# tum-pbs/Solver-in-the-Loop

Measured on AMD Instinct MI355X. Metric: sim-steps/s, SOL-32 training (karman-2d 128x64, fwd+bwd+Adam), higher is better.
Workload: dtype f32 (fp16x3 split MFMA in 32-ch convs); 1 GPU; karman-2d 128x64 SOL-32, batch 6 Re values per GPU (BASELINE configs[2]); global_batch=6, msteps=32, parallelism=dp1

## Files before the change

solver-in-the-loop_amd/csrc/conv5x5.hip:

```cpp
#include "common.hpp"
#include <stdlib.h>

namespace {

typedef float f32x4 __attribute__((ext_vector_type(4)));

__host__ __device__ inline int pad_in(int c) { return c <= 4 ? 4 : 32; }
__host__ __device__ inline int pad_out(int c) { return c <= 16 ? 16 : 32; }

__global__ void k_pack(const float* __restrict__ w, float* __restrict__ packed, int cin, int cout, int mode) {
    const int IP = pad_in(cin), OP = pad_out(cout);
    const int total = 25 * OP * IP;
    for (int e = blockIdx.x * blockDim.x + threadIdx.x; e < total; e += gridDim.x * blockDim.x) {
        const int i = e % IP, o = (e / IP) % OP, tap = e / (IP * OP);
        float v = 0.f;
        if (i < cin && o < cout) {
            if (mode == SOL_CONV_FWD) v = w[(tap * cin + i) * cout + o];
            else v = w[((24 - tap) * cout + o) * cin + i];
        }
        packed[e] = v;
    }
}

template <int CIN, int NT, bool MASK = false>
// ... 707 lines not shown
    __syncthreads();
    while (gr < gr_end) {
        const int gnext = next_row(gr + 1);
        if (gnext < gr_end) load_row(gnext);
        const bool valid = row_valid(gr);
        const float* xs = smem + cur * bufsz;
        const float* zs = xs + (W + 4) * CPX;
        if (active_wave) {
            for (int p0 = 0; p0 < W; p0 += 4) {
                const int px = p0 + g;
                float bv;
                if constexpr (COUT > 4) bv = zs[px * CPZ + tc * 16 + li];
                else bv = li < 4 ? zs[px * CPZ + li] : 0.f;
                if (dy == 2 && ta == 0) bsum += bv;
                if (valid) {
#pragma unroll
                    for (int d = 0; d < 5; ++d) {
                        float av;
                        if constexpr (CI == 32) av = xs[(px + d) * CPX + ta * 16 + li];
                        else av = li < 4 ? xs[(px + d) * CPX + li] : 0.f;
                        acc[d] = __builtin_amdgcn_mfma_f32_16x16x4f32(av, bv, acc[d], 0, 0, 0);
                    }
                }
            }
        }
        if (gnext < gr_end) store_row(smem + (cur ^ 1) * bufsz);
        __syncthreads();
        cur ^= 1;
        gr = gnext;
    }
    if (!active_wave) return;
    float* pw = a.partial + (size_t)blk * (25 * IP * OP);
#pragma unroll
    for (int d = 0; d < 5; ++d) {
        const int tap = dy * 5 + d;
#pragma unroll
        for (int r = 0; r < 4; ++r) {
            const int ci = ta * 16 + 4 * g + r, co = tc * 16 + li;
            float* dst = &pw[(tap * IP + ci) * OP + co];
            *dst = a.overwrite ? acc[d][r] : *dst + acc[d][r];
        }
    }
    if (dy == 2 && ta == 0) {
        bsum += __shfl_xor(bsum, 16, 64);
        bsum += __shfl_xor(bsum, 32, 64);
        if (g == 0) {
            float* pb = a.partial + (size_t)a.nblk * (25 * IP * OP) + (size_t)blk * OP;
            pb[tc * 16 + li] = a.overwrite ? bsum : pb[tc * 16 + li] + bsum;
        }
    }
}

typedef float f32x16 __attribute__((ext_vector_type(16)));

__global__ void __launch_bounds__(256) k_conv5x5_bww32(BwArgs a) {
    constexpr int W = 64, STG = (W + 4) * 32 + W * 32;
    extern __shared__ __align__(16) float smem[];
    const int tid = threadIdx.x, lane = tid & 63, wave = tid >> 6;
    const int c = lane & 31, kpx = lane >> 5;
    const int H = a.H;
    const int dy = blockIdx.x % 5, blk = blockIdx.x / 5;
    f32x16 acc[5];
#pragma unroll
    for (int d = 0; d < 5; ++d)
#pragma unroll
        for (int r = 0; r < 16; ++r) acc[d][r] = 0.f;
    float bsum = 0.f;
    const int R = a.nseg * a.B * H, RPS = a.B * H;
    const int gr_end = min((blk + 1) * a.rb, R);
    auto row_valid = [&](int gr) { const int y = gr % H, yy = y + dy - 2; return yy >= 0 && yy < H; };
    auto next_row = [&](int gr) { while (gr < gr_end && !(dy == 2 || row_valid(gr))) ++gr; return gr; };
    float4 xr[3], zr[2];
    auto load_row = [&](int gr) {
        const int seg = gr / RPS, grs = gr - seg * RPS;
        const int b = grs / H, y = grs - b * H, yy = y + dy - 2;
        const bool valid = yy >= 0 && yy < H;
        const float4* gx = reinterpret_cast<const float4*>(a.x + (size_t)seg * a.x_seg) + (size_t)(b * H + (valid ? yy : 0)) * W * 8;
#pragma unroll
        for (int n = 0; n < 3; ++n) {
            const int e = tid + n * 256, px = e >> 3, c4 = e & 7, xx = px - 2;
            xr[n] = make_float4(0.f, 0.f, 0.f, 0.f);
            if (valid && px < W + 4 && xx >= 0 && xx < W) xr[n] = gx[xx * 8 + c4];
        }
        const float4* gz = reinterpret_cast<const float4*>(a.dz + (size_t)seg * a.dz_seg) + (size_t)(b * H + y) * W * 8;
#pragma unroll
        for (int n = 0; n < 2; ++n) zr[n] = gz[tid + n * 256];
    };
    auto store_row = [&](float* buf) {
#pragma unroll
        for (int n = 0; n < 3; ++n) {
            const int e = tid + n * 256;
            if (e < (W + 4) * 8) reinterpret_cast<float4*>(buf)[e] = xr[n];
        }
        float4* zs4 = reinterpret_cast<float4*>(buf + (W + 4) * 32);
#pragma unroll
        for (int n = 0; n < 2; ++n) zs4[tid + n * 256] = zr[n];
    };
    int gr = next_row(blk * a.rb);
    int cur = 0;
    if (gr < gr_end) { load_row(gr); store_row(smem); }
    __syncthreads();
    while (gr < gr_end) {
        const int gnext = next_row(gr + 1);
        if (gnext < gr_end) load_row(gnext);
        const bool valid = row_valid(gr);
        const float* xs = smem + cur * STG + (16 * wave + kpx) * 32 + c;
        const float* zs = smem + cur * STG + (W + 4) * 32 + (16 * wave + kpx) * 32 + c;
#pragma unroll
        for (int ks = 0; ks < 8; ++ks) {
            const float bv = zs[ks * 64];
            if (dy == 2) bsum += bv;
            if (valid) {
#pragma unroll
                for (int d = 0; d < 5; ++d)
                    acc[d] = __builtin_amdgcn_mfma_f32_32x32x2f32(xs[(2 * ks + d) * 32], bv, acc[d], 0, 0, 0);
            }
        }
        if (gnext < gr_end) store_row(smem + (cur ^ 1) * STG);
        __syncthreads();
        cur ^= 1;
        gr = gnext;
    }
    float* red = smem;
    float* pw = a.partial + (size_t)blk * (25 * 1024);
    for (int d = 0; d < 5; ++d) {
#pragma unroll
        for (int r = 0; r < 16; ++r) {
            const int row = (r & 3) + 8 * (r >> 2) + 4 * kpx;
            red[wave * 1024 + row * 32 + c] = acc[d][r];
        }
        __syncthreads();
#pragma unroll
        for (int n = 0; n < 4; ++n) {
            const int idx = tid + n * 256;
            const float v = (red[idx] + red[1024 + idx]) + (red[2048 + idx] + red[3072 + idx]);
            float* dst = &pw[(dy * 5 + d) * 1024 + idx];
            *dst = a.overwrite ? v : *dst + v;
        }
        __syncthreads();
    }
    if (dy == 2) {
        bsum += __shfl_xor(bsum, 32, 64);
        if (kpx == 0) red[wave * 32 + c] = bsum;
        __syncthreads();
        if (tid < 32) {
            float* pb = a.partial + (size_t)a.nblk * (25 * 1024) + (size_t)blk * 32;
            const float v = (red[tid] + red[32 + tid]) + (red[64 + tid] + red[96 + tid]);
            pb[tid] = a.overwrite ? v : pb[tid] + v;
        }
    }
}

template <int MODE, int MT, bool WIDE = false>
__global__ void __launch_bounds__(256) k_conv5x5_bww_thin(BwArgs a) {
    constexpr int W = 64;
    constexpr int XC = MODE == 0 ? 4 : 32, ZC = MODE == 0 ? 32 : 2;
    constexpr int XROWS = MODE == 0 ? 5 : 1, ZROWS = MODE == 0 ? 1 : 5;
    constexpr int XSZ = (W + 4) * XC;
    constexpr int ZSZ = (MODE == 0 ? W + 4 : W + 8) * ZC;
    constexpr int STG = XROWS * XSZ + ZROWS * ZSZ;
    constexpr int IP = MODE == 0 ? 16 : 32, OP = MODE == 0 ? 32 : 16;
    constexpr int XF4 = XROWS * XSZ / 4, ZF4 = ZROWS * ZSZ / 4;
    constexpr int NXR = (XF4 + 255) / 256, NZR = (ZF4 + 255) / 256;
    constexpr int NTM = MODE == 0 ? MT : 2, NTN = MODE == 0 ? 2 : 1;
    constexpr int CI0 = MT == 1 ? 3 : 4;
    typedef float bt_f4 __attribute__((ext_vector_type(4)));
    extern __shared__ __align__(16) float smem[];
    const int tid = threadIdx.x, lane = tid & 63, wave = tid >> 6;
    const int n16 = lane & 15, kq = lane >> 4;
    const int H = a.H, blk = blockIdx.x;
    const int WI = WIDE ? a.W : W, tiles = WIDE ? a.W / W : 1;
    const int rblk = WIDE ? blk / tiles : blk, x0 = WIDE ? (blk - rblk * tiles) * W : 0;
    bt_f4 acc[5][NTM][NTN];
#pragma unroll
    for (int d = 0; d < 5; ++d)
#pragma unroll
        for (int tm = 0; tm < NTM; ++tm)
#pragma unroll
            for (int tn = 0; tn < NTN; ++tn) acc[d][tm][tn] = (bt_f4){0.f, 0.f, 0.f, 0.f};
    float bsum[2] = {0.f, 0.f};
    const int R = a.nseg * a.B * H, RPS = a.B * H;
    const int gr_end = min((rblk + 1) * a.rb, R);
    float4 xr[NXR], zr[NZR];
    auto load_row = [&](int gr) {
        const int seg = gr / RPS, grs = gr - seg * RPS;
        const int b = grs / H, y = grs - b * H;
        const float* xb = a.x + (size_t)seg * a.x_seg + (size_t)b * H * WI * XC;
        const float* zb = a.dz + (size_t)seg * a.dz_seg + ((size_t)b * H * WI + x0) * ZC;
#pragma unroll
        for (int n = 0; n < NXR; ++n) {
            const int e = tid + n * 256;
            xr[n] = make_float4(0.f, 0.f, 0.f, 0.f);
            if (e < XF4) {
                const int row = e / (XSZ / 4), f = e - row * (XSZ / 4);
                const int px = f / (XC / 4), c4 = f - px * (XC / 4), xx = x0 + px - 2;
                const int yy = MODE == 0 ? y + row - 2 : y;
                if (yy >= 0 && yy < H && xx >= 0 && xx < WI) xr[n] = reinterpret_cast<const float4*>(xb + ((size_t)yy * WI + xx) * XC)[c4];
            }
        }
#pragma unroll
        for (int n = 0; n < NZR; ++n) {
            const int e = tid + n * 256;
            zr[n] = make_float4(0.f, 0.f, 0.f, 0.f);
            if (e < ZF4) {
                if (MODE == 0) {
                    if (e < W * ZC / 4) zr[n] = reinterpret_cast<const float4*>(zb + (size_t)y * WI * ZC)[e];
                } else {
                    const int row = e / (ZSZ / 4), f = e - row * (ZSZ / 4);
                    const int yy = y + 2 - row, p = 2 * f - 4;
                    if (yy >= 0 && yy < H && p >= 0 && p < W) zr[n] = reinterpret_cast<const float4*>(zb + ((size_t)yy * WI + p) * ZC)[0];
                }
            }
        }
    };
    auto store_row = [&](float* buf) {
#pragma unroll
        for (int n = 0; n < NXR; ++n) { const int e = tid + n * 256; if (e < XF4) reinterpret_cast<float4*>(buf)[e] = xr[n]; }
#pragma unroll
        for (int n = 0; n < NZR; ++n) { const int e = tid + n * 256; if (e < ZF4) reinterpret_cast<float4*>(buf + XROWS * XSZ)[e] = zr[n]; }
    };
    int gr = rblk * a.rb, cur = 0;
    if (gr < gr_end) { load_row(gr); store_row(smem); }
    __syncthreads();
    for (; gr < gr_end; ++gr) {
        if (gr + 1 < gr_end) load_row(gr + 1);
        const float* xs = smem + cur * STG;
        const float* zs = xs + XROWS * XSZ;
        if (MODE == 0) {
            int aoff[NTM];
            bool aok[NTM];
#pragma unroll
            for (int tm = 0; tm < NTM; ++tm) {
                const int i = 16 * tm + n16;
                aok[tm] = i < 5 * CI0;
                aoff[tm] = aok[tm] ? (i / CI0) * 4 + i % CI0 : 0;
            }
#pragma unroll
            for (int ks = 0; ks < 4; ++ks) {
                const int px = 16 * wave + 4 * ks + kq;
                float bv[2];
#pragma unroll
                for (int tn = 0; tn < 2; ++tn) { bv[tn] = zs[px * 32 + 16 * tn + n16]; bsum[tn] += bv[tn]; }
#pragma unroll
                for (int d = 0; d < 5; ++d) {
#pragma unroll
                    for (int tm = 0; tm < NTM; ++tm) {
                        const float av = aok[tm] ? xs[d * XSZ + px * 4 + aoff[tm]] : 0.f;
#pragma unroll
                        for (int tn = 0; tn < NTN; ++tn) acc[d][tm][tn] = __builtin_amdgcn_mfma_f32_16x16x4f32(av, bv[tn], acc[d][tm][tn], 0, 0, 0);
                    }
                }
            }
        } else {
            const int dxi = n16 >> 1, co = n16 & 1;
#pragma unroll
            for (int ks = 0; ks < 5; ++ks) {
                const int g = wave + 4 * ks;
                const bool ok = g < 17;
                const int qq = ok ? 4 * g + kq : 0;
                float av[2];
#pragma unroll
                for (int tm = 0; tm < 2; ++tm) av[tm] = ok ? xs[qq * 32 + 16 * tm + n16] : 0.f;
#pragma unroll
                for (int d = 0; d < 5; ++d) {
                    const float bv = (ok && n16 < 10) ? zs[d * ZSZ + (qq - dxi + 4) * 2 + co] : 0.f;
                    if (d == 2 && n16 < 2) bsum[0] += bv;
#pragma unroll
                    for (int tm = 0; tm < 2; ++tm) acc[d][tm][0] = __builtin_amdgcn_mfma_f32_16x16x4f32(av[tm], bv, acc[d][tm][0], 0, 0, 0);
                }
            }
        }
        if (gr + 1 < gr_end) store_row(smem + (cur ^ 1) * STG);
        __syncthreads();
        cur ^= 1;
    }
    float* red = smem;
    float* pw = a.partial + (size_t)blk * (25 * IP * OP);
    for (int d = 0; d < 5; ++d) {
#pragma unroll
        for (int tm = 0; tm < NTM; ++tm)
#pragma unroll
            for (int tn = 0; tn < NTN; ++tn)
#pragma unroll
                for (int r = 0; r < 4; ++r) red[wave * 1024 + (16 * tm + 4 * kq + r) * 32 + 16 * tn + n16] = acc[d][tm][tn][r];
        __syncthreads();
#pragma unroll
        for (int n = 0; n < 4; ++n) {
            const int idx = tid + n * 256, row = idx >> 5, col = idx & 31;
            const float v = (red[idx] + red[1024 + idx]) + (red[2048 + idx] + red[3072 + idx]);
            int tap, ci, co;
            bool keep;
            if (MODE == 0) { tap = d * 5 + row / CI0; ci = row % CI0; co = col; keep = row < 5 * CI0; }
            else { tap = d * 5 + (col >> 1); ci = row; co = col & 1; keep = col < 10; }
            if (keep) {
                float* dst = &pw[(tap * IP + ci) * OP + co];
                *dst = a.overwrite ? v : *dst + v;
            }
        }
        __syncthreads();
    }
    {
#pragma unroll
        for (int t = 0; t < 2; ++t) {
            bsum[t] += __shfl_xor(bsum[t], 16, 64);
            bsum[t] += __shfl_xor(bsum[t], 32, 64);
            if (kq == 0) red[wave * 32 + 16 * t + n16] = bsum[t];
        }
        __syncthreads();
        const int nb = MODE == 0 ? 32 : 2;
        if (tid < nb) {
            float* pb = a.partial + (size_t)a.nblk * (25 * IP * OP) + (size_t)blk * OP;
            const float v = (red[tid] + red[32 + tid]) + (red[64 + tid] + red[96 + tid]);
            pb[tid] = a.overwrite ? v : pb[tid] + v;
        }
    }
}

__global__ void k_bww_reduce(float* __restrict__ partial, float* __restrict__ dw, float* __restrict__ db,
                             int nblk, int cin, int cout, int IP, int OP, int chunk, int stride, int to_dw, int accumulate, int tt) {
    const int nw = 25 * cin * cout;
    const int e = blockIdx.x * blockDim.x + threadIdx.x;
    const int k0 = blockIdx.y * chunk * stride, k1 = min(k0 + chunk * stride, nblk);
    if (e < nw) {
        const int co = e % cout, ci = (e / cout) % cin, tap = e / (cout * cin);
        const size_t off = (size_t)(tap * IP + ci) * OP + co;
        float s = 0.f;
        for (int k = k0; k < k1; k += stride) s += partial[(size_t)k * (25 * IP * OP) + off];
        const int eo = tt ? (((tap % 5) * 5 + tap / 5) * cin + ci) * cout + co : e;
        if (to_dw) dw[eo] = accumulate ? dw[eo] + s : s;
        else partial[(size_t)k0 * (25 * IP * OP) + off] = s;
    } else if (e < nw + cout) {
        const int co = e - nw;
        float* pb = partial + (size_t)nblk * (25 * IP * OP);
        float s = 0.f;
        for (int k = k0; k < k1; k += stride) s += pb[(size_t)k * OP + co];
        if (to_dw) db[co] = accumulate ? db[co] + s : s;
        else pb[(size_t)k0 * OP + co] = s;
    }
}

struct ReduceJob { float *partial, *dw, *db; int nblk, cin, cout, IP, OP, ny, accumulate, tt; };
struct ReduceJobs { ReduceJob j[12]; };
__global__ void k_bww_reduce_jobs(ReduceJobs J, int stage2) {
    const ReduceJob& r = J.j[blockIdx.z];
    constexpr int CHUNK = 16;
    const int nw = 25 * r.cin * r.cout;
    const int e = blockIdx.x * blockDim.x + threadIdx.x;
    int k0, k1, stride, to_dw;
    if (!stage2) {
        if (r.ny <= 1 || (int)blockIdx.y >= r.ny) return;
        k0 = blockIdx.y * CHUNK; k1 = min(k0 + CHUNK, r.nblk); stride = 1; to_dw = 0;
    } else {
        if (blockIdx.y > 0) return;
        k0 = 0; k1 = r.nblk; stride = r.ny > 1 ? CHUNK : 1; to_dw = 1;
    }
    if (e < nw) {
        const int co = e % r.cout, ci = (e / r.cout) % r.cin, tap = e / (r.cout * r.cin);
        const size_t off = (size_t)(tap * r.IP + ci) * r.OP + co;
        float s = 0.f;
        for (int k = k0; k < k1; k += stride) s += r.partial[(size_t)k * (25 * r.IP * r.OP) + off];
        const int eo = r.tt ? (((tap % 5) * 5 + tap / 5) * r.cin + ci) * r.cout + co : e;
        if (to_dw) r.dw[eo] = r.accumulate ? r.dw[eo] + s : s;
        else r.partial[(size_t)k0 * (25 * r.IP * r.OP) + off] = s;
    } else if (e < nw + r.cout) {
        const int co = e - nw;
        float* pb = r.partial + (size_t)r.nblk * (25 * r.IP * r.OP);
        float s = 0.f;
        for (int k = k0; k < k1; k += stride) s += pb[(size_t)k * r.OP + co];
        if (to_dw) r.db[co] = r.accumulate ? r.db[co] + s : s;
        else pb[(size_t)k0 * r.OP + co] = s;
    }
}

int check_shape(int B, int H, int W, int cin, int cout) {
    SOL_REQUIRE(B >= 1 && H >= 1 && W >= 4, "conv5x5: bad image shape B=%d H=%d W=%d", B, H, W);
    SOL_REQUIRE((W <= 64 && 64 % W == 0 && H % (64 / W) == 0) || W % 64 == 0,
                "conv5x5: W must divide 64 (with H %% (64/W) == 0) or be a multiple of 64 (H=%d W=%d)", H, W);
    SOL_REQUIRE(cin == 4 || cin == 32, "conv5x5: input channels must be 4 (zero padded) or 32 (got %d)", cin);
    SOL_REQUIRE(cout >= 1 && cout <= 32, "conv5x5: output channels must be in [1,32] (got %d)", cout);
    return SOL_OK;
}

}

extern "C" int32_t sol_absmax_slots(void) {
    static_assert(SOL_AMAX_SLOTS == SOL_ABSMAX_SLOTS, "include/sol_hip.h and common.hpp disagree");
    return SOL_AMAX_SLOTS;
}

extern "C" size_t sol_conv5x5_packed_floats(int32_t cin, int32_t cout, int32_t ) {
    return (size_t)25 * pad_in(cin) * pad_out(cout) +
           (pad_in(cin) == 32 ? sol_conv_sb_packed_floats(pad_out(cout)) + sol_conv_sh_packed_floats(pad_out(cout)) : 0);
}

extern "C" int sol_conv5x5_pack(void* stream, const float* w_hwio, int32_t cin, int32_t cout, int32_t mode, float* packed) {
    SOL_REQUIRE(w_hwio && packed, "sol_conv5x5_pack: NULL pointer");
    SOL_REQUIRE(cin >= 1 && cin <= 32 && cout >= 1 && cout <= 32, "sol_conv5x5_pack: channels out of range");
    SOL_REQUIRE(mode == SOL_CONV_FWD || mode == SOL_CONV_BWD_DATA, "sol_conv5x5_pack: bad mode %d", mode);
    const int total = 25 * pad_in(cin) * pad_out(cout);
    SOL_LAUNCH(k_pack, dim3((total + 255) / 256), dim3(256), 0, (hipStream_t)stream, w_hwio, packed, cin, cout, mode);
    SOL_LAUNCH_CHECK();
    if (pad_in(cin) == 32) {
        if (int e = sol_conv_sb_pack((hipStream_t)stream, w_hwio, cin, cout, mode, packed + total)) return e;
        return sol_conv_sh_pack((hipStream_t)stream, w_hwio, cin, cout, mode, packed + total + sol_conv_sb_packed_floats(pad_out(cout)));
    }
    return SOL_OK;
}

extern "C" int sol_conv5x5_pack_jobs(void* stream, int32_t n, const float* const* w_hwio, const int32_t* cin, const int32_t* cout,
                                     const int32_t* mode, float* const* packed) {
    SOL_REQUIRE(n >= 1 && n <= 24 && w_hwio && cin && cout && mode && packed, "sol_conv5x5_pack_jobs: 1 <= n <= 24 jobs, no NULL array");
    const float* bi[24];
    float* bo[24];
    int ci[24], co[24], md[24];
    for (int k = 0; k < n; ++k) {
        SOL_REQUIRE(w_hwio[k] && packed[k], "sol_conv5x5_pack_jobs: NULL pointer in job %d", k);
        SOL_REQUIRE(cin[k] >= 1 && cin[k] <= 32 && cout[k] >= 1 && cout[k] <= 32, "sol_conv5x5_pack_jobs: channels out of range in job %d", k);
        SOL_REQUIRE(mode[k] == SOL_CONV_FWD || mode[k] == SOL_CONV_BWD_DATA, "sol_conv5x5_pack_jobs: bad mode %d in job %d", mode[k], k);
        bi[k] = nullptr; bo[k] = nullptr; ci[k] = cin[k]; co[k] = cout[k]; md[k] = mode[k];
    }
    return sol_pack_jobs((hipStream_t)stream, n, w_hwio, packed, bo, bi, ci, co, md, 0);
}

int sol_init_conv_kernels() {
    static std::atomic<unsigned long long> optin{0};
    return sol_lds_optin(optin, {SOL_K(k_conv5x5_r3<1>), SOL_K(k_conv5x5_r3<2>), SOL_K(k_conv5x5_c32<1>), SOL_K(k_conv5x5_c32<2>),
                                 SOL_K((k_conv5x5_r3<1, true>)), SOL_K((k_conv5x5_r3<2, true>)), SOL_K((k_conv5x5_c32<1, true>)), SOL_K((k_conv5x5_c32<2, true>))}, "conv kernels");
}

static int conv_impl(void* stream, const float* x, const float* packed, const float* bias,
                     const float* residual, const float* act_ref, float* y,
                     int32_t B, int32_t H, int32_t W, int32_t cin, int32_t cout,
                     int32_t epilogue, float slope, const uint32_t* x_absmax, uint32_t* y_absmax, int32_t WV = 0) {
    if (int e = check_shape(B, H, W, cin, cout)) return e;
    SOL_REQUIRE(x && packed && y, "sol_conv5x5: NULL pointer");
    SOL_REQUIRE(epilogue != SOL_EPI_DLRELU || act_ref, "sol_conv5x5: SOL_EPI_DLRELU needs act_ref");
    if (int e = sol_init_conv_kernels()) return e;
    ConvArgs a{};
    a.x = x; a.wp = packed; a.bias = bias; a.res = residual; a.act = act_ref; a.y = y;
    a.B = B; a.H = H; a.W = W; a.CO = cout; a.CI = cin; a.epi = epilogue; a.slope = slope; a.WV = WV;
    const bool mask = sol_conv_masked(a);
    a.TW = W < 64 ? W : 64;
    a.RPW = 64 / a.TW;
    a.tiles_x = W / a.TW;
    const int grid = B * (H / a.RPW) * a.tiles_x;
    const int CP = cin == 4 ? 4 : 36;
    size_t lds = (size_t)(a.RPW + 4) * (a.TW + 4) * CP * sizeof(float);
    if (cin == 4) {
        lds += (size_t)25 * pad_out(cout) * 4 * sizeof(float);
        if (lds < 4 * 16 * 32 * sizeof(float)) lds = 4 * 16 * 32 * sizeof(float);
    }
    const int NT = pad_out(cout) / 16;
    hipStream_t s = (hipStream_t)stream;
    const bool use_sb = sol_opt().conv_precision != 2;
    const bool use_sh = sol_opt().conv_precision == 0;
    if (use_sb) a.ymax = y_absmax;
    if (cin == 32 && W % 64 == 0 && use_sb) {
        a.wsb = packed + (size_t)25 * 32 * pad_out(cout);
        a.wsh = packed + (size_t)25 * 32 * pad_out(cout) + sol_conv_sb_packed_floats(pad_out(cout));
        a.xmax = use_sh ? x_absmax : nullptr;
        return sol_conv_sb_launch(s, a, NT, B * H * (W / 64));
    }
    if (cin == 32 && W % 64 == 0 && sol_opt().conv_r3) {
        const int ntiles = B * H * (W / 64);
        const size_t ldsr = ((size_t)3 * 2 * 68 * 32 + 2 * (size_t)5 * NT * 16 * 32) * sizeof(float);
        const int grid3 = (ntiles + 2) / 3;
        if (mask) {
            if (NT == 2) SOL_LAUNCH((k_conv5x5_r3<2, true>), dim3(grid3), dim3(768), ldsr, s, a, ntiles);
            else SOL_LAUNCH((k_conv5x5_r3<1, true>), dim3(grid3), dim3(768), ldsr, s, a, ntiles);
        } else if (NT == 2) {
            SOL_LAUNCH((k_conv5x5_r3<2>), dim3(grid3), dim3(768), ldsr, s, a, ntiles);
        } else {
            SOL_LAUNCH((k_conv5x5_r3<1>), dim3(grid3), dim3(768), ldsr, s, a, ntiles);
        }
    }
    else if (cin == 32) {
        const size_t lds32 = ((size_t)(a.RPW + 4) * (a.TW + 4) * 32 + 2 * (size_t)NT * 16 * 32) * sizeof(float);
        if (mask) {
            if (NT == 2) SOL_LAUNCH((k_conv5x5_c32<2, true>), dim3(grid), dim3(256), lds32, s, a);
            else SOL_LAUNCH((k_conv5x5_c32<1, true>), dim3(grid), dim3(256), lds32, s, a);
        } else if (NT == 2) {
            SOL_LAUNCH((k_conv5x5_c32<2>), dim3(grid), dim3(256), lds32, s, a);
        } else {
            SOL_LAUNCH((k_conv5x5_c32<1>), dim3(grid), dim3(256), lds32, s, a);
        }
    }
    else if (conv_t3_usable(B, H, W, cin, pad_out(cout)) && cout == pad_out(cout)) {
        if (mask) {
            if (NT == 2) SOL_LAUNCH((k_conv5x5_t3<2, true>), dim3((B * H + 2) / 3), dim3(768), conv_t3_lds(32), s, a);
            else SOL_LAUNCH((k_conv5x5_t3<1, true>), dim3((B * H + 2) / 3), dim3(768), conv_t3_lds(16), s, a);
        }
        else if (NT == 2) SOL_LAUNCH((k_conv5x5_t3<2>), dim3((B * H + 2) / 3), dim3(768), conv_t3_lds(32), s, a);
        else SOL_LAUNCH((k_conv5x5_t3<1>), dim3((B * H + 2) / 3), dim3(768), conv_t3_lds(16), s, a);
    }
    else if (mask) {
        if (NT == 2) SOL_LAUNCH((k_conv5x5<4, 2, true>), dim3(grid), dim3(256), lds, s, a);
        else SOL_LAUNCH((k_conv5x5<4, 1, true>), dim3(grid), dim3(256), lds, s, a);
    }
    else if (cin == 4 && NT == 2) SOL_LAUNCH((k_conv5x5<4, 2>), dim3(grid), dim3(256), lds, s, a);
    else SOL_LAUNCH((k_conv5x5<4, 1>), dim3(grid), dim3(256), lds, s, a);
    SOL_LAUNCH_CHECK();
    return SOL_OK;
}

extern "C" int sol_conv5x5(void* stream, const float* x, const float* packed, const float* bias,
                           const float* residual, const float* act_ref, float* y,
                           int32_t B, int32_t H, int32_t W, int32_t cin, int32_t cout,
                           int32_t epilogue, float slope) {
    return conv_impl(stream, x, packed, bias, residual, act_ref, y, B, H, W, cin, cout, epilogue, slope, nullptr, nullptr);
}

const void* sol_conv_packed_wsh(const float* packed, int cout) {
    return packed + (size_t)25 * 32 * pad_out(cout) + sol_conv_sb_packed_floats(pad_out(cout));
}

int sol_conv5x5_seed(void* stream, const float* packed_bwd, const float* act_ref, float* y, int B, int H, int W, float slope, unsigned* y_absmax,
                     const float* vy, const float* vx, const float* gt_vy, const float* gt_vx, const float* gin_vy, const float* gin_vx,
                     float* g_vy, float* g_vx, float* dO2, float s0, float s1, float l0, float l1, float inv_m) {
    if (int e = check_shape(B, H, W, 4, 32)) return e;
    SOL_REQUIRE(W == 64 && packed_bwd && act_ref && y && vy && vx && gt_vy && gt_vx && g_vy && g_vx && dO2 && !gin_vy == !gin_vx, "sol_conv5x5_seed: bad arguments");
    if (int e = sol_init_conv_kernels()) return e;
    ConvArgs a{};
    a.x = nullptr; a.wp = packed_bwd; a.act = act_ref; a.y = y;
// ... 68 lines not shown
extern "C" size_t sol_conv5x5_bwd_weight_ws_floats(int32_t B, int32_t H, int32_t W, int32_t cin, int32_t cout) {
    int nblk, IP, OP;
    bww_dims(B * H, RB, cin, cout, &nblk, &IP, &OP, bww_tiles(W));
    return (size_t)nblk * (25 * IP * OP + OP);
}

int sol_bww_pick_rb(int rows) { return pick_rb(rows); }

size_t sol_bww_batched_ws_floats(int nseg, int B, int H, int cin, int cout) {
    int nblk, IP, OP;
    const int rows = nseg * B * H;
    bww_dims(rows, pick_rb(rows, cin, cout), cin, cout, &nblk, &IP, &OP);
    return (size_t)nblk * (25 * IP * OP + OP);
}

static int bww_launch(void* stream, const float* x, const float* dz, float* partial, int nseg, long x_seg, long dz_seg,
                      int rb, int overwrite, int B, int H, int W, int cin, int cout, int nblk_layout = 0,
                      const unsigned* xmax = nullptr, const unsigned* zmax = nullptr, long xmax_seg = 0, long zmax_seg = 0, int cin_real = 0) {
    SOL_REQUIRE(x && dz && partial, "sol_conv5x5_bwd_weight: NULL pointer");
    SOL_REQUIRE(B >= 1 && H >= 1 && W >= 4 && W % 4 == 0, "sol_conv5x5_bwd_weight: need W >= 4, W %% 4 == 0 (got %d)", W);
    SOL_REQUIRE(W <= 64 || W % 64 == 0, "sol_conv5x5_bwd_weight: rows wider than 64 pixels must be a multiple of 64 pixels wide (got W = %d)", W);
    SOL_REQUIRE(W <= 64 || (nblk_layout == 0 && nseg == 1), "sol_conv5x5_bwd_weight: the batched forms take W <= 64 (got %d)", W);
    const int tiles = bww_tiles(W), Wt = W > 64 ? 64 : W;
    SOL_REQUIRE((cin == 4 || cin == 32) && (cout == 2 || cout == 32),
                "sol_conv5x5_bwd_weight: supported (cin,cout) are {4,32}x{2,32} (got %d,%d)", cin, cout);
    BwArgs a{};
    a.x = x; a.dz = dz; a.partial = partial; a.B = B; a.H = H; a.W = W; a.cin = cin; a.cout = cout;
    a.nseg = nseg; a.rb = rb; a.x_seg = x_seg; a.dz_seg = dz_seg; a.overwrite = overwrite;
    a.xmax = xmax; a.zmax = zmax; a.xmax_seg = xmax_seg; a.zmax_seg = zmax_seg; a.cin_real = cin_real;
    int IP, OP;
    bww_dims(nseg * B * H, rb, cin, cout, &a.nblk, &IP, &OP, tiles);
    const int nblk_run = a.nblk;
    if (nblk_layout > 0) a.nblk = nblk_layout;
    const int CPX = cin == 4 ? 4 : 48, CPZ = cout <= 4 ? 4 : 48;
    const size_t lds = 2 * ((size_t)(Wt + 4) * CPX + (size_t)Wt * CPZ) * sizeof(float);
    const int grid = nblk_run * 5;
    hipStream_t s = (hipStream_t)stream;
    if (W > 64 && ((cin == 4 && cout == 32) || (cin == 32 && cout == 2)) && sol_opt().conv_thin) {
        if (cin == 4) {
            const size_t l0 = 2 * (size_t)(5 * 68 * 4 + 68 * 32) * sizeof(float);
            if (a.cin_real >= 1 && a.cin_real <= 3) SOL_LAUNCH((k_conv5x5_bww_thin<0, 1, true>), dim3(nblk_run), dim3(256), l0, s, a);
            else SOL_LAUNCH((k_conv5x5_bww_thin<0, 2, true>), dim3(nblk_run), dim3(256), l0, s, a);
        } else {
            const size_t l1 = 2 * (size_t)(68 * 32 + 5 * 72 * 2) * sizeof(float);
            SOL_LAUNCH((k_conv5x5_bww_thin<1, 2, true>), dim3(nblk_run), dim3(256), l1, s, a);
        }
        SOL_LAUNCH_CHECK();
        return SOL_OK;
    }
    if (W == 64 && ((cin == 4 && cout == 32) || (cin == 32 && cout == 2)) && sol_opt().conv_thin) {
        if (cin == 4) {
            const size_t l0 = 2 * (size_t)(5 * 68 * 4 + 68 * 32) * sizeof(float);
            if (a.cin_real >= 1 && a.cin_real <= 3) SOL_LAUNCH((k_conv5x5_bww_thin<0, 1>), dim3(nblk_run), dim3(256), l0, s, a);
            else SOL_LAUNCH((k_conv5x5_bww_thin<0, 2>), dim3(nblk_run), dim3(256), l0, s, a);
        } else {
            const size_t l1 = 2 * (size_t)(68 * 32 + 5 * 72 * 2) * sizeof(float);
            SOL_LAUNCH((k_conv5x5_bww_thin<1, 2>), dim3(nblk_run), dim3(256), l1, s, a);
        }
        SOL_LAUNCH_CHECK();
        return SOL_OK;
    }
    if (cin == 32 && cout == 32 && W % 64 == 0 && sol_opt().conv_precision != 2) return sol_bww_sb_launch(s, a, nblk_run);
    if (cin == 32 && cout == 32 && W == 64 && sol_opt().conv_bww32) {
        const size_t lds3 = 2 * ((size_t)(64 + 4) * 32 + 64 * 32) * sizeof(float);
        SOL_LAUNCH(k_conv5x5_bww32, dim3(grid), dim3(256), lds3, s, a);
    }
    else if (cin == 32 && cout == 32) SOL_LAUNCH((k_conv5x5_bww<32, 32>), dim3(grid), dim3(256), lds, s, a);
    else if (cin == 32 && cout == 2) SOL_LAUNCH((k_conv5x5_bww<32, 2>), dim3(grid), dim3(256), lds, s, a);
    else if (cin == 4 && cout == 32) SOL_LAUNCH((k_conv5x5_bww<4, 32>), dim3(grid), dim3(256), lds, s, a);
    else SOL_LAUNCH((k_conv5x5_bww<4, 2>), dim3(grid), dim3(256), lds, s, a);
    SOL_LAUNCH_CHECK();
    return SOL_OK;
}

extern "C" int sol_conv5x5_bwd_weight(void* stream, const float* x, const float* dz, float* partial,
                                      int32_t B, int32_t H, int32_t W, int32_t cin, int32_t cout) {
    return bww_launch(stream, x, dz, partial, 1, 0, 0, RB, 0, B, H, W, cin, cout);
}

int sol_bww_batched(void* stream, const float* x, const float* dz, float* partial, int nseg, int nseg_layout, int overwrite,
                    long x_seg, long dz_seg, int B, int H, int W, int cin, int cout,
                    const unsigned* xmax, const unsigned* zmax, long xmax_seg, long zmax_seg, int cin_real) {
    const int rb = pick_rb(nseg_layout * B * H, cin, cout);
    int nblk, IP, OP;
    bww_dims(nseg_layout * B * H, rb, cin, cout, &nblk, &IP, &OP);
    return bww_launch(stream, x, dz, partial, nseg, x_seg, dz_seg, rb, overwrite, B, H, W, cin, cout, nblk, xmax, zmax, xmax_seg, zmax_seg, cin_real);
}

int sol_bww_batched_jobs(void* stream, int n, const float* const* x, const float* const* dz, float* const* partial, const int* nplanes, int overwrite,
                         int H, int W, const unsigned* xmax, const unsigned* zmax, int rb) {
    SOL_REQUIRE(n >= 1 && n <= 5 && W == 64 && H >= 1 && sol_opt().conv_precision != 2, "sol_bww_batched_jobs: 1..5 jobs of the split kernels, W == 64");
    BwJobs p{};
    p.n = n;
    for (int k = 0; k < n; ++k) {
        SOL_REQUIRE(x[k] && dz[k] && partial[k] && nplanes[k] >= 1, "sol_bww_batched_jobs: bad job %d", k);
        BwArgs& a = p.a[k];
        a.x = x[k]; a.dz = dz[k]; a.partial = partial[k]; a.B = nplanes[k]; a.H = H; a.W = W; a.cin = 32; a.cout = 32;
        a.nseg = 1; a.rb = rb > 0 ? rb : pick_rb(nplanes[k] * H); a.x_seg = 0;
        SOL_REQUIRE(a.rb >= pick_rb(nplanes[k] * H), "sol_bww_batched_jobs: %d rows per workgroup is below the layout's %d", a.rb, pick_rb(nplanes[k] * H)); a.dz_seg = 0; a.overwrite = overwrite;
        a.xmax = xmax; a.zmax = zmax; a.xmax_seg = 0; a.zmax_seg = 0; a.cin_real = 0;
        int IP, OP;
        bww_dims(nplanes[k] * H, a.rb, 32, 32, &a.nblk, &IP, &OP);
        p.nrun[k] = a.nblk;
        p.wg_per = p.wg_per > a.nblk ? p.wg_per : a.nblk;
    }
    return sol_bww_sb_jobs_launch((hipStream_t)stream, p);
}

static int bww_reduce(void* stream, const float* partial, float* dw_hwio, float* db, int rows, int rb, int cin, int cout, int accumulate, int tt = 0, int tiles = 1) {
    SOL_REQUIRE(partial && dw_hwio && db, "sol_conv5x5_bwd_weight_reduce: NULL pointer");
    SOL_REQUIRE(cin >= 1 && cin <= 32 && cout >= 1 && cout <= 32, "sol_conv5x5_bwd_weight_reduce: channels out of range");
    int nblk, IP, OP;
    bww_dims(rows, rb, cin <= 4 ? 4 : 32, cout, &nblk, &IP, &OP, tiles);
    const int total = 25 * cin * cout + cout;
    float* pm = const_cast<float*>(partial);
    const int chunk = 16, ny = (nblk + chunk - 1) / chunk;
    hipStream_t hs = (hipStream_t)stream;
    if (ny > 1) {
        SOL_LAUNCH(k_bww_reduce, dim3((total + 255) / 256, ny), dim3(256), 0, hs, pm, dw_hwio, db, nblk, cin, cout, IP, OP, chunk, 1, 0, 0, 0);
        SOL_LAUNCH_CHECK();
        SOL_LAUNCH(k_bww_reduce, dim3((total + 255) / 256, 1), dim3(256), 0, hs, pm, dw_hwio, db, nblk, cin, cout, IP, OP, ny, chunk, 1, accumulate, tt);
    } else {
        SOL_LAUNCH(k_bww_reduce, dim3((total + 255) / 256, 1), dim3(256), 0, hs, pm, dw_hwio, db, nblk, cin, cout, IP, OP, nblk, 1, 1, accumulate, tt);
    }
    SOL_LAUNCH_CHECK();
    return SOL_OK;
}

extern "C" int sol_conv5x5_bwd_weight_reduce(void* stream, const float* partial, float* dw_hwio, float* db,
                                             int32_t B, int32_t H, int32_t W, int32_t cin, int32_t cout,
                                             int32_t accumulate) {
    SOL_REQUIRE(W <= 64 || W % 64 == 0, "sol_conv5x5_bwd_weight_reduce: rows wider than 64 pixels must be a multiple of 64 pixels wide (got W = %d)", W);
    return bww_reduce(stream, partial, dw_hwio, db, B * H, RB, cin, cout, accumulate, 0, bww_tiles(W));
}

size_t sol_bww_step_ws_floats(int B, int H, int rb) { return (size_t)((B * H) / rb) * (25 * 32 * 32 + 32); }

int sol_bww_step_job(BwArgs* out, const float* x, const float* dz, float* partial, int overwrite, int B, int H, int W, int rb,
                     const unsigned* xmax, const unsigned* zmax) {
    SOL_REQUIRE(out && x && dz && partial && xmax && zmax, "sol_bww_step_job: NULL pointer");
    SOL_REQUIRE(W == 64 && rb >= 1 && (B * H) % rb == 0, "sol_bww_step_job: W == 64 and rb | B*H required (W=%d, B*H=%d, rb=%d)", W, B * H, rb);
    BwArgs a{};
    a.x = x; a.dz = dz; a.partial = partial; a.B = B; a.H = H; a.W = W; a.cin = 32; a.cout = 32;
    a.nblk = (B * H) / rb; a.nseg = 1; a.rb = rb; a.x_seg = 0; a.dz_seg = 0; a.overwrite = overwrite;
    a.xmax = xmax; a.zmax = zmax; a.xmax_seg = 0; a.zmax_seg = 0;
    *out = a;
    return SOL_OK;
}

int sol_bww_reduce_layers(void* stream, int n, float* const* partial, float* const* dw_hwio, float* const* db, const int* rows, const int* rb,
                          const int* cin, const int* cout, int accumulate, int taps_transposed, int tiles) {
    SOL_REQUIRE(n >= 1 && n <= 12, "sol_bww_reduce_layers: 1 <= n <= 12");
    ReduceJobs J{};
    int max_total = 0, max_ny = 1;
    for (int i = 0; i < n; ++i) {
        SOL_REQUIRE(partial[i] && dw_hwio[i] && db[i] && cin[i] >= 1 && cin[i] <= 32 && cout[i] >= 1 && cout[i] <= 32, "sol_bww_reduce_layers: bad layer %d", i);
        ReduceJob& r = J.j[i];
        const int rbi = rb[i] > 0 ? rb[i] : pick_rb(rows[i], cin[i] <= 4 ? 4 : 32, cout[i]);
        bww_dims(rows[i], rbi, cin[i] <= 4 ? 4 : 32, cout[i], &r.nblk, &r.IP, &r.OP, tiles);
        r.partial = partial[i]; r.dw = dw_hwio[i]; r.db = db[i]; r.cin = cin[i]; r.cout = cout[i];
        r.ny = (r.nblk + 15) / 16; r.accumulate = accumulate; r.tt = taps_transposed;
        max_total = max_total > 25 * cin[i] * cout[i] + cout[i] ? max_total : 25 * cin[i] * cout[i] + cout[i];
        max_ny = max_ny > r.ny ? max_ny : r.ny;
    }
    hipStream_t hs = (hipStream_t)stream;
    if (max_ny > 1) {
        SOL_LAUNCH(k_bww_reduce_jobs, dim3((max_total + 255) / 256, max_ny, n), dim3(256), 0, hs, J, 0);
        SOL_LAUNCH_CHECK();
    }
    SOL_LAUNCH(k_bww_reduce_jobs, dim3((max_total + 255) / 256, 1, n), dim3(256), 0, hs, J, 1);
    SOL_LAUNCH_CHECK();
    return SOL_OK;
}

extern "C" int sol_conv5x5_bwd_weight_reduce_jobs(void* stream, int32_t n, float* const* partial, float* const* dw_hwio, float* const* db,
                                                  int32_t B, int32_t H, int32_t W, const int32_t* cin, const int32_t* cout, int32_t accumulate) {
    SOL_REQUIRE(n >= 1 && n <= 12 && partial && dw_hwio && db && cin && cout && B >= 1 && H >= 1, "sol_conv5x5_bwd_weight_reduce_jobs: 1 <= n <= 12 layers, no NULL array");
    SOL_REQUIRE(W <= 64 || W % 64 == 0, "sol_conv5x5_bwd_weight_reduce_jobs: rows wider than 64 pixels must be a multiple of 64 pixels wide (got W = %d)", W);
    int rows[12], rb[12], ci[12], co[12];
    for (int k = 0; k < n; ++k) { rows[k] = B * H; rb[k] = RB; ci[k] = cin[k]; co[k] = cout[k]; }
    return sol_bww_reduce_layers(stream, n, partial, dw_hwio, db, rows, rb, ci, co, accumulate, 0, bww_tiles(W));
}

extern "C" size_t sol_conv5x5_bwd_weight_segments_ws_floats(int32_t nseg, int32_t B, int32_t H, int32_t cin, int32_t cout) {
    if (nseg < 1 || B < 1 || H < 1) return 0;
    return sol_bww_batched_ws_floats(nseg, B, H, cin, cout);
}

extern "C" int sol_conv5x5_bwd_weight_segments(void* stream, const float* x, const float* dz, float* partial, int32_t nseg, int64_t x_seg, int64_t dz_seg,
                                               int32_t overwrite, int32_t B, int32_t H, int32_t W, int32_t cin, int32_t cout,
                                               const uint32_t* x_absmax, const uint32_t* dz_absmax, int64_t absmax_seg, int32_t cin_real) {
    SOL_REQUIRE(nseg >= 1, "sol_conv5x5_bwd_weight_segments: nseg must be at least 1 (got %d)", nseg);
    SOL_REQUIRE(W <= 64, "sol_conv5x5_bwd_weight_segments: the segmented form takes rows of W <= 64 pixels (got W = %d)", W);
    SOL_REQUIRE(x_seg >= 0 && dz_seg >= 0 && absmax_seg >= 0, "sol_conv5x5_bwd_weight_segments: negative segment stride");
    SOL_REQUIRE(cin_real >= 0 && cin_real <= cin, "sol_conv5x5_bwd_weight_segments: cin_real must lie in [0, cin] (got %d, cin = %d)", cin_real, cin);
    return sol_bww_batched(stream, x, dz, partial, nseg, nseg, overwrite ? 1 : 0, (long)x_seg, (long)dz_seg, B, H, W, cin, cout,
                           x_absmax, dz_absmax, (long)absmax_seg, (long)absmax_seg, cin_real);
}

extern "C" int sol_conv5x5_bwd_weight_segments_reduce(void* stream, float* partial, float* dw_hwio, float* db, int32_t nseg, int32_t B, int32_t H,
                                                      int32_t cin, int32_t cout, int32_t accumulate) {
    SOL_REQUIRE(partial && dw_hwio && db, "sol_conv5x5_bwd_weight_segments_reduce: NULL pointer");
    SOL_REQUIRE(nseg >= 1 && B >= 1 && H >= 1, "sol_conv5x5_bwd_weight_segments_reduce: nseg, B, H must be at least 1 (got %d, %d, %d)", nseg, B, H);
    float* parts[1] = {partial}; float* dws[1] = {dw_hwio}; float* dbs[1] = {db};
    const int rows[1] = {nseg * B * H}, rbs[1] = {0}, ci[1] = {cin}, co[1] = {cout};
    return sol_bww_reduce_layers(stream, 1, parts, dws, dbs, rows, rbs, ci, co, accumulate, 0, 1);
}

int sol_bww_step_reduce(void* stream, const float* partial, float* dw_hwio, float* db, int B, int H, int rb, int cin, int cout, int accumulate) {
    return bww_reduce(stream, partial, dw_hwio, db, B * H, rb, cin, cout, accumulate);
}

int sol_bww_batched_reduce(void* stream, const float* partial, float* dw_hwio, float* db, int nseg, int B, int H,
                           int cin, int cout, int accumulate, int taps_transposed) {
    const int rows = nseg * B * H;
    return bww_reduce(stream, partial, dw_hwio, db, rows, pick_rb(rows, cin <= 4 ? 4 : 32, cout), cin, cout, accumulate, taps_transposed);
}
```

Baseline: 17350 sim-steps/s.

## Deepen thin weight-grad prefetch pipeline and fuse two-pass partial reduction

The thin backward-weight conv kernel now precomputes clamped load offsets, issues unconditional clamped global loads up to two rows ahead, and masks invalid elements at staging time. It also uses branchless bitmask zeroing, a double-buffered LDS read schedule in MODE 1, and explicit lgkmcnt barriers plus occupancy launch bounds. The two-launch partial reduction is replaced by a single launch in which several threads per element sum chunks and combine them through shared memory. The aim is to hide global load latency, cut divergent branches, and remove one kernel launch and the intermediate write-back. The cost is more register pressure and extra clamped redundant loads.

Result: no change. 17420 sim-steps/s (median of 6 runs) (+0.4%).

```diff
diff --git a/solver-in-the-loop_amd/csrc/conv5x5.hip b/solver-in-the-loop_amd/csrc/conv5x5.hip
--- a/solver-in-the-loop_amd/csrc/conv5x5.hip
+++ b/solver-in-the-loop_amd/csrc/conv5x5.hip
@@ -883,7 +883,7 @@
 }
 
 template <int MODE, int MT, bool WIDE = false>
-__global__ void __launch_bounds__(256) k_conv5x5_bww_thin(BwArgs a) {
+__global__ void __launch_bounds__(256, MT == 2 && MODE == 0 ? 2 : 4) k_conv5x5_bww_thin(BwArgs a) {
     constexpr int W = 64;
     constexpr int XC = MODE == 0 ? 4 : 32, ZC = MODE == 0 ? 32 : 2;
     constexpr int XROWS = MODE == 0 ? 5 : 1, ZROWS = MODE == 0 ? 1 : 5;
@@ -893,6 +893,8 @@
     constexpr int IP = MODE == 0 ? 16 : 32, OP = MODE == 0 ? 32 : 16;
     constexpr int XF4 = XROWS * XSZ / 4, ZF4 = ZROWS * ZSZ / 4;
     constexpr int NXR = (XF4 + 255) / 256, NZR = (ZF4 + 255) / 256;
+    constexpr int NS = MODE == 0 ? 2 : 1;
+    constexpr int NZQ = MODE == 0 ? W * ZC / 4 / 256 : NZR;
     constexpr int NTM = MODE == 0 ? MT : 2, NTN = MODE == 0 ? 2 : 1;
     constexpr int CI0 = MT == 1 ? 3 : 4;
     typedef float bt_f4 __attribute__((ext_vector_type(4)));
@@ -911,59 +913,72 @@
             for (int tn = 0; tn < NTN; ++tn) acc[d][tm][tn] = (bt_f4){0.f, 0.f, 0.f, 0.f};
     float bsum[2] = {0.f, 0.f};
     const int R = a.nseg * a.B * H, RPS = a.B * H;
-    const int gr_end = min((rblk + 1) * a.rb, R);
-    float4 xr[NXR], zr[NZR];
-    auto load_row = [&](int gr) {
-        const int seg = gr / RPS, grs = gr - seg * RPS;
-        const int b = grs / H, y = grs - b * H;
+    const int r0 = rblk * a.rb, gr_end = min(r0 + a.rb, R);
+    int xdy[NXR], xo[NXR], zdy[NZR], zo[NZR];
+    bool xok[NXR], zok[NZR];
+#pragma unroll
+    for (int n = 0; n < NXR; ++n) {
+        const int e = tid + n * 256, ec = min(e, XF4 - 1);
+        const int row = ec / (XSZ / 4), f = ec - row * (XSZ / 4);
+        const int px = f / (XC / 4), c4 = f - px * (XC / 4), xx = x0 + px - 2;
+        xdy[n] = MODE == 0 ? row - 2 : 0;
+        xok[n] = e < XF4 && xx >= 0 && xx < WI;
+        xo[n] = min(max(xx, 0), WI - 1) * XC + c4 * 4;
+    }
+#pragma unroll
+    for (int n = 0; n < NZR; ++n) {
+        const int e = tid + n * 256, ec = min(e, ZF4 - 1);
+        if (MODE == 0) {
+            zdy[n] = 0;
+            zok[n] = e < W * ZC / 4;
+            zo[n] = min(e, W * ZC / 4 - 1) * 4;
+        } else {
+            const int row = ec / (ZSZ / 4), f = ec - row * (ZSZ / 4);
+            const int p = 2 * f - 4;
+            zdy[n] = 2 - row;
+            zok[n] = e < ZF4 && p >= 0 && p < W;
+            zo[n] = min(max(p, 0), W - 2) * ZC;
+        }
+    }
+    auto request = [&](int gr, bt_f4 (&xr)[NXR], bt_f4 (&zr)[NZQ], int& y) __attribute__((always_inline)) {
+        const int rr = gr < gr_end ? gr : min(r0, R - 1);
+        const int seg = rr / RPS, grs = rr - seg * RPS;
+        const int b = grs / H;
+        y = grs - b * H;
         const float* xb = a.x + (size_t)seg * a.x_seg + (size_t)b * H * WI * XC;
         const float* zb = a.dz + (size_t)seg * a.dz_seg + ((size_t)b * H * WI + x0) * ZC;
 #pragma unroll
+        for (int n = 0; n < NXR; ++n)
+            xr[n] = *reinterpret_cast<const bt_f4*>(xb + (unsigned)(min(max(y + xdy[n], 0), H - 1) * (WI * XC) + xo[n]));
+#pragma unroll
+        for (int n = 0; n < NZQ; ++n)
+            zr[n] = *reinterpret_cast<const bt_f4*>(zb + (unsigned)(min(max(y + zdy[n], 0), H - 1) * (WI * ZC) + zo[n]));
+    };
+    auto stage = [&](const bt_f4 (&xr)[NXR], const bt_f4 (&zr)[NZQ], int y, float* buf) __attribute__((always_inline)) {
+        const bt_f4 zero = {0.f, 0.f, 0.f, 0.f};
+#pragma unroll
         for (int n = 0; n < NXR; ++n) {
-            const int e = tid + n * 256;
-            xr[n] = make_float4(0.f, 0.f, 0.f, 0.f);
-            if (e < XF4) {
-                const int row = e / (XSZ / 4), f = e - row * (XSZ / 4);
-                const int px = f / (XC / 4), c4 = f - px * (XC / 4), xx = x0 + px - 2;
-                const int yy = MODE == 0 ? y + row - 2 : y;
-                if (yy >= 0 && yy < H && xx >= 0 && xx < WI) xr[n] = reinterpret_cast<const float4*>(xb + ((size_t)yy * WI + xx) * XC)[c4];
-            }
+            const int e = tid + n * 256, yy = y + xdy[n];
+            if (e < XF4) reinterpret_cast<bt_f4*>(buf)[e] = (xok[n] && yy >= 0 && yy < H) ? xr[n] : zero;
         }
 #pragma unroll
         for (int n = 0; n < NZR; ++n) {
-            const int e = tid + n * 256;
-            zr[n] = make_float4(0.f, 0.f, 0.f, 0.f);
-            if (e < ZF4) {
-                if (MODE == 0) {
-                    if (e < W * ZC / 4) zr[n] = reinterpret_cast<const float4*>(zb + (size_t)y * WI * ZC)[e];
-                } else {
-                    const int row = e / (ZSZ / 4), f = e - row * (ZSZ / 4);
-                    const int yy = y + 2 - row, p = 2 * f - 4;
-                    if (yy >= 0 && yy < H && p >= 0 && p < W) zr[n] = reinterpret_cast<const float4*>(zb + ((size_t)yy * WI + p) * ZC)[0];
-                }
-            }
+            const int e = tid + n * 256, yy = y + zdy[n];
+            if (e < ZF4) reinterpret_cast<bt_f4*>(buf + XROWS * XSZ)[e] = (n < NZQ && zok[n] && yy >= 0 && yy < H) ? zr[n < NZQ ? n : 0] : zero;
         }
     };
-    auto store_row = [&](float* buf) {
-#pragma unroll
-        for (int n = 0; n < NXR; ++n) { const int e = tid + n * 256; if (e < XF4) reinterpret_cast<float4*>(buf)[e] = xr[n]; }
-#pragma unroll
-        for (int n = 0; n < NZR; ++n) { const int e = tid + n * 256; if (e < ZF4) reinterpret_cast<float4*>(buf + XROWS * XSZ)[e] = zr[n]; }
-    };
-    int gr = rblk * a.rb, cur = 0;
-    if (gr < gr_end) { load_row(gr); store_row(smem); }
-    __syncthreads();
-    for (; gr < gr_end; ++gr) {
-        if (gr + 1 < gr_end) load_row(gr + 1);
-        const float* xs = smem + cur * STG;
+    auto masked = [](float v, unsigned m) { return __uint_as_float(__float_as_uint(v) & m); };
+    auto mfma_row = [&](const float* xs) __attribute__((always_inline)) {
         const float* zs = xs + XROWS * XSZ;
         if (MODE == 0) {
             int aoff[NTM];
+            unsigned amask[NTM];
             bool aok[NTM];
 #pragma unroll
             for (int tm = 0; tm < NTM; ++tm) {
                 const int i = 16 * tm + n16;
                 aok[tm] = i < 5 * CI0;
+                amask[tm] = aok[tm] ? ~0u : 0u;
                 aoff[tm] = aok[tm] ? (i / CI0) * 4 + i % CI0 : 0;
             }
 #pragma unroll
@@ -976,35 +991,73 @@
                 for (int d = 0; d < 5; ++d) {
 #pragma unroll
                     for (int tm = 0; tm < NTM; ++tm) {
-                        const float av = aok[tm] ? xs[d * XSZ + px * 4 + aoff[tm]] : 0.f;
+                        const float av = masked(xs[d * XSZ + px * 4 + aoff[tm]], amask[tm]);
 #pragma unroll
                         for (int tn = 0; tn < NTN; ++tn) acc[d][tm][tn] = __builtin_amdgcn_mfma_f32_16x16x4f32(av, bv[tn], acc[d][tm][tn], 0, 0, 0);
                     }
                 }
             }
         } else {
-            const int dxi = n16 >> 1, co = n16 & 1;
+            const int dxi = min(n16 >> 1, 4), co = n16 & 1;
+            const unsigned bmask = n16 < 10 ? ~0u : 0u, w0mask = wave == 0 ? ~0u : 0u;
+            const int q0 = 4 * wave + kq, q4 = wave == 0 ? 64 + kq : 0;
+            const float* const xa = xs + q0 * 32 + n16;
+            const float* const za = zs + (q0 - dxi + 4) * 2 + co;
+            const float* const xa4 = xs + q4 * 32 + n16;
+            const float* const za4 = zs + (q4 - dxi + 4) * 2 + co;
+            float av[2][2], bv[2][5];
+            auto read_step = [&](int ks, float (&a2)[2], float (&b5)[5]) __attribute__((always_inline)) {
+#pragma unroll
+                for (int tm = 0; tm < 2; ++tm) a2[tm] = ks < 4 ? xa[ks * 512 + 16 * tm] : masked(xa4[16 * tm], w0mask);
+#pragma unroll
+                for (int d = 0; d < 5; ++d)
+                    b5[d] = ks < 4 ? masked(za[d * ZSZ + ks * 32], bmask) : masked(za4[d * ZSZ], bmask & w0mask);
+            };
+            read_step(0, av[0], bv[0]);
 #pragma unroll
             for (int ks = 0; ks < 5; ++ks) {
-                const int g = wave + 4 * ks;
-                const bool ok = g < 17;
-                const int qq = ok ? 4 * g + kq : 0;
-                float av[2];
-#pragma unroll
-                for (int tm = 0; tm < 2; ++tm) av[tm] = ok ? xs[qq * 32 + 16 * tm + n16] : 0.f;
+                if (ks < 4) read_step(ks + 1, av[(ks + 1) & 1], bv[(ks + 1) & 1]);
 #pragma unroll
                 for (int d = 0; d < 5; ++d) {
-                    const float bv = (ok && n16 < 10) ? zs[d * ZSZ + (qq - dxi + 4) * 2 + co] : 0.f;
-                    if (d == 2 && n16 < 2) bsum[0] += bv;
-#pragma unroll
-                    for (int tm = 0; tm < 2; ++tm) acc[d][tm][0] = __builtin_amdgcn_mfma_f32_16x16x4f32(av[tm], bv, acc[d][tm][0], 0, 0, 0);
+                    if (d == 2 && n16 < 2) bsum[0] += bv[ks & 1][d];
+#pragma unroll
+                    for (int tm = 0; tm < 2; ++tm) acc[d][tm][0] = __builtin_amdgcn_mfma_f32_16x16x4f32(av[ks & 1][tm], bv[ks & 1][d], acc[d][tm][0], 0, 0, 0);
                 }
-            }
-        }
-        if (gr + 1 < gr_end) store_row(smem + (cur ^ 1) * STG);
-        __syncthreads();
-        cur ^= 1;
-    }
+                __builtin_amdgcn_sched_barrier(0);
+            }
+        }
+    };
+#define BT_BARRIER() asm volatile("s_waitcnt lgkmcnt(0)\n\ts_barrier" ::: "memory")
+    bt_f4 xA[NXR], zA[NZQ], xB[NXR], zB[NZQ];
+    int yA, yB = 0;
+#pragma unroll
+    for (int n = 0; n < NXR; ++n) xB[n] = (bt_f4){0.f, 0.f, 0.f, 0.f};
+#pragma unroll
+    for (int n = 0; n < NZQ; ++n) zB[n] = (bt_f4){0.f, 0.f, 0.f, 0.f};
+    {
+        bt_f4 xP[NXR], zP[NZQ];
+        int yP;
+        request(r0, xP, zP, yP);
+        request(r0 + 1, xA, zA, yA);
+        if (NS == 2) request(r0 + 2, xB, zB, yB);
+        __builtin_amdgcn_sched_barrier(0);
+        if (r0 < gr_end) stage(xP, zP, yP, smem);
+    }
+    BT_BARRIER();
+    auto do_row = [&](int gr, int cur, bt_f4 (&xs_)[NXR], bt_f4 (&zs_)[NZQ], int& ys_) __attribute__((always_inline)) {
+        if (gr + 1 < gr_end) stage(xs_, zs_, ys_, smem + (cur ^ 1) * STG);
+        request(gr + 1 + NS, xs_, zs_, ys_);
+        __builtin_amdgcn_sched_barrier(0);
+        mfma_row(smem + cur * STG);
+        BT_BARRIER();
+    };
+    for (int gr = r0; gr < gr_end; gr += 2) {
+        do_row(gr, 0, xA, zA, yA);
+        if (gr + 1 >= gr_end) break;
+        if (NS == 2) do_row(gr + 1, 1, xB, zB, yB);
+        else do_row(gr + 1, 1, xA, zA, yA);
+    }
+#undef BT_BARRIER
     float* red = smem;
     float* pw = a.partial + (size_t)blk * (25 * IP * OP);
     for (int d = 0; d < 5; ++d) {
@@ -1070,36 +1123,44 @@
     }
 }
 
-struct ReduceJob { float *partial, *dw, *db; int nblk, cin, cout, IP, OP, ny, accumulate, tt; };
+struct ReduceJob { float *partial, *dw, *db; int nblk, cin, cout, IP, OP, ny, accumulate, tt, lanes; };
 struct ReduceJobs { ReduceJob j[12]; };
-__global__ void k_bww_reduce_jobs(ReduceJobs J, int stage2) {
-    const ReduceJob& r = J.j[blockIdx.z];
+__global__ void __launch_bounds__(256) k_bww_reduce_jobs(ReduceJobs J) {
+    const ReduceJob& r = J.j[blockIdx.y];
     constexpr int CHUNK = 16;
+    __shared__ float sums[256];
+    const int lanes = r.lanes, epb = 256 / lanes;
     const int nw = 25 * r.cin * r.cout;
-    const int e = blockIdx.x * blockDim.x + threadIdx.x;
-    int k0, k1, stride, to_dw;
-    if (!stage2) {
-        if (r.ny <= 1 || (int)blockIdx.y >= r.ny) return;
-        k0 = blockIdx.y * CHUNK; k1 = min(k0 + CHUNK, r.nblk); stride = 1; to_dw = 0;
+    if ((int)blockIdx.x * epb >= nw + r.cout) return;
+    const int el = threadIdx.x % epb, cl = threadIdx.x / epb;
+    const int e = blockIdx.x * epb + el;
+    const bool is_w = e < nw, live = e < nw + r.cout;
+    const int co = is_w ? e % r.cout : e - nw, ci = is_w ? (e / r.cout) % r.cin : 0, tap = is_w ? e / (r.cout * r.cin) : 0;
+    const float* src = is_w ? r.partial + (size_t)(tap * r.IP + ci) * r.OP + co : r.partial + (size_t)r.nblk * (25 * r.IP * r.OP) + co;
+    const size_t sstride = is_w ? (size_t)25 * r.IP * r.OP : (size_t)r.OP;
+    float total = 0.f;
+    for (int c0 = 0; c0 < r.ny; c0 += lanes) {
+        const int c = c0 + cl;
+        float s = 0.f;
+        if (live && c < r.ny) {
+            const int k1 = min(c * CHUNK + CHUNK, r.nblk);
+            for (int k = c * CHUNK; k < k1; ++k) s += src[(size_t)k * sstride];
+        }
+        if (lanes == 1) { total += s; continue; }
+        sums[cl * epb + el] = s;
+        __syncthreads();
+        if (cl == 0) {
+            const int n = min(lanes, r.ny - c0);
+            for (int q = 0; q < n; ++q) total += sums[q * epb + el];
+        }
+        __syncthreads();
+    }
+    if (!live || cl != 0) return;
+    if (is_w) {
+        const int eo = r.tt ? (((tap % 5) * 5 + tap / 5) * r.cin + ci) * r.cout + co : e;
+        r.dw[eo] = r.accumulate ? r.dw[eo] + total : total;
     } else {
-        if (blockIdx.y > 0) return;
-        k0 = 0; k1 = r.nblk; stride = r.ny > 1 ? CHUNK : 1; to_dw = 1;
-    }
-    if (e < nw) {
-        const int co = e % r.cout, ci = (e / r.cout) % r.cin, tap = e / (r.cout * r.cin);
-        const size_t off = (size_t)(tap * r.IP + ci) * r.OP + co;
-        float s = 0.f;
-        for (int k = k0; k < k1; k += stride) s += r.partial[(size_t)k * (25 * r.IP * r.OP) + off];
-        const int eo = r.tt ? (((tap % 5) * 5 + tap / 5) * r.cin + ci) * r.cout + co : e;
-        if (to_dw) r.dw[eo] = r.accumulate ? r.dw[eo] + s : s;
-        else r.partial[(size_t)k0 * (25 * r.IP * r.OP) + off] = s;
-    } else if (e < nw + r.cout) {
-        const int co = e - nw;
-        float* pb = r.partial + (size_t)r.nblk * (25 * r.IP * r.OP);
-        float s = 0.f;
-        for (int k = k0; k < k1; k += stride) s += pb[(size_t)k * r.OP + co];
-        if (to_dw) r.db[co] = r.accumulate ? r.db[co] + s : s;
-        else pb[(size_t)k0 * r.OP + co] = s;
+        r.db[co] = r.accumulate ? r.db[co] + total : total;
     }
 }
 
@@ -1474,7 +1535,7 @@
                           const int* cin, const int* cout, int accumulate, int taps_transposed, int tiles) {
     SOL_REQUIRE(n >= 1 && n <= 12, "sol_bww_reduce_layers: 1 <= n <= 12");
     ReduceJobs J{};
-    int max_total = 0, max_ny = 1;
+    int grid_x = 1;
     for (int i = 0; i < n; ++i) {
         SOL_REQUIRE(partial[i] && dw_hwio[i] && db[i] && cin[i] >= 1 && cin[i] <= 32 && cout[i] >= 1 && cout[i] <= 32, "sol_bww_reduce_layers: bad layer %d", i);
         ReduceJob& r = J.j[i];
@@ -1482,15 +1543,11 @@
         bww_dims(rows[i], rbi, cin[i] <= 4 ? 4 : 32, cout[i], &r.nblk, &r.IP, &r.OP, tiles);
         r.partial = partial[i]; r.dw = dw_hwio[i]; r.db = db[i]; r.cin = cin[i]; r.cout = cout[i];
         r.ny = (r.nblk + 15) / 16; r.accumulate = accumulate; r.tt = taps_transposed;
-        max_total = max_total > 25 * cin[i] * cout[i] + cout[i] ? max_total : 25 * cin[i] * cout[i] + cout[i];
-        max_ny = max_ny > r.ny ? max_ny : r.ny;
-    }
-    hipStream_t hs = (hipStream_t)stream;
-    if (max_ny > 1) {
-        SOL_LAUNCH(k_bww_reduce_jobs, dim3((max_total + 255) / 256, max_ny, n), dim3(256), 0, hs, J, 0);
-        SOL_LAUNCH_CHECK();
-    }
-    SOL_LAUNCH(k_bww_reduce_jobs, dim3((max_total + 255) / 256, 1, n), dim3(256), 0, hs, J, 1);
+        for (r.lanes = 1; r.lanes < 32 && r.lanes < r.ny;) r.lanes *= 2;
+        const int total = 25 * cin[i] * cout[i] + cout[i], epb = 256 / r.lanes;
+        grid_x = std::max(grid_x, (total + epb - 1) / epb);
+    }
+    SOL_LAUNCH(k_bww_reduce_jobs, dim3(grid_x, n), dim3(256), 0, (hipStream_t)stream, J);
     SOL_LAUNCH_CHECK();
     return SOL_OK;
 }
```
